# psipred/DMPfold2

Hardware: AMD Instinct MI355X
Metric: structures/s at L=300, N_seq=2000, 10 iters+100 min (higher is better)
Workload: dtype f32 with full-width operands on the bf16 matrix cores (option precision = 2): convolution operands split exactly into 3 bf16 pieces (24 significand bits), the 6 piece products above 2^-24 accumulated in f32 by v_mfma_f32_32x32x16_bf16; vertical GRU the same way (3 bf16 pieces per operand, 6 products

## Files before the change

### dmpfold2_amd/csrc/conv_bf16.h

```cpp
#pragma once
#include "common.h"
#include <vector>

namespace dmp {

typedef float cq_f32x16 __attribute__((ext_vector_type(16)));
typedef __bf16 cq_bf16x8 __attribute__((ext_vector_type(8)));

#ifndef CQ_PITCH_N
#define CQ_PITCH_N 20
#endif
constexpr int CQ_PITCH = CQ_PITCH_N;
constexpr int CQ_HCOLS = 20;
template <int NQ> struct CqShape {
  static constexpr int ROWS = 2 * NQ;
  static constexpr int HALO = ROWS + 4;
  static constexpr int RP = ROWS + 3;
  static constexpr int PIECE = 2 * HALO * CQ_PITCH;
  static constexpr int IN_SLOTS = 3 * PIECE;
  static constexpr int IN_PAD = (IN_SLOTS + 63) / 64 * 64;
  static constexpr int IN_BYTES = IN_PAD * 16;
};
constexpr int CQ_WSLOT = 3 * 2 * 32;
constexpr int CQ_WCOL = 5 * CQ_WSLOT;
constexpr int CQ_WBUF = 3 * CQ_WSLOT;
template <int NQ> constexpr int convq_lds_bytes() { return CqShape<NQ>::IN_BYTES + 4 * CQ_WBUF * 16; }
constexpr int CONVQ_LDS_BYTES = convq_lds_bytes<8>();

__host__ __device__ inline uint16_t cq_bf16_rne(float f) {
  uint32_t u = __builtin_bit_cast(uint32_t, f);
  u += 0x7FFFu + ((u >> 16) & 1u);
  return (uint16_t)(u >> 16);
}
__host__ __device__ inline float cq_bf16_f32(uint16_t h) {
  return __builtin_bit_cast(float, (uint32_t)h << 16);
}
__host__ __device__ inline void split3_bf16(float x, uint16_t p[3]) {
  p[0] = cq_bf16_rne(x);
  const float r1 = x - cq_bf16_f32(p[0]);
  p[1] = cq_bf16_rne(r1);
  const float r2 = r1 - cq_bf16_f32(p[1]);
  p[2] = cq_bf16_rne(r2);
}

inline std::vector<uint16_t> pack_conv_weights_bf16(const float* w) {
  const int tap_row[5] = {0, 2, 4, 1, 3};
  std::vector<uint16_t> q((size_t)4 * 8 * 25 * 4 * 3 * 2 * 32 * 8);
  for (int split = 0; split < 4; ++split)
    for (int g = 0; g < 8; ++g)
      for (int dx = 0; dx < 5; ++dx)
        for (int wave = 0; wave < 4; ++wave)
          for (int sl = 0; sl < 5; ++sl)
            for (int cg = 0; cg < 2; ++cg)
              for (int m = 0; m < 32; ++m)
                for (int e = 0; e < 8; ++e) {
                  const int oc = split * 128 + wave * 32 + m, ic = g * 16 + cg * 8 + e;
                  uint16_t p3[3];
                  split3_bf16(w[((size_t)oc * 128 + ic) * 25 + tap_row[sl] * 5 + dx], p3);
                  for (int p = 0; p < 3; ++p)
                    q[(((((((((size_t)split * 8 + g) * 5 + dx) * 4 + wave) * 5 + sl) * 3 + p) * 2 + cg) * 32 + m) * 8) + e] = p3[p];
                }
  return q;
}

#if defined(__HIPCC__) && defined(CONV_BF16_KERNELS)
__device__ __forceinline__ void cq_dma16(const void* gsrc, unsigned lds_byte_addr) {
  unsigned keep;
  asm volatile("s_mov_b32 %0, m0\n\ts_mov_b32 m0, %2\n\ts_nop 0\n\tglobal_load_lds_dwordx4 %1, off\n\ts_mov_b32 m0, %0"
               : "=&s"(keep) : "v"(gsrc), "s"(lds_byte_addr) : "memory");
}
template <int N> __device__ __forceinline__ void cq_wait_vm() {
  asm volatile("s_waitcnt vmcnt(%0)" :: "n"(N) : "memory");
}

__device__ __forceinline__ cq_f32x16 cq_mfma(uint4 a, uint4 b, cq_f32x16 c) {
  return __builtin_amdgcn_mfma_f32_32x32x16_bf16(__builtin_bit_cast(cq_bf16x8, a),
                                                 __builtin_bit_cast(cq_bf16x8, b), c, 0, 0, 0);
}

__device__ __forceinline__ void cq_lane_pixel(int li, int& row, int& x) {
  const bool a = li < 4 || (li >= 12 && li < 16) || (li >= 20 && li < 28);
  row = a ? 0 : 1;
  if (a) x = li < 4 ? li : (li < 16 ? li - 8 : li - 12);
  else x = li < 12 ? li - 4 : (li < 20 ? li - 8 : li - 16);
}

template <int NQ, int NT, int PAR>
__device__ __forceinline__ void cq_column_pass(const uint4 (&a)[NT][3], const uint4* il, cq_f32x16 (&acc)[NQ]) {
  constexpr int PIECE = CqShape<NQ>::PIECE, RP = CqShape<NQ>::RP;
  uint4 bn0 = il[PAR * CQ_PITCH], bn1 = il[PAR * CQ_PITCH + PIECE], bn2 = il[PAR * CQ_PITCH + 2 * PIECE];
#pragma unroll
  for (int r = PAR; r < RP; r += 2) {
    const uint4 b0 = bn0, b1 = bn1, b2 = bn2;
    if (r + 2 < RP) {
      bn0 = il[(r + 2) * CQ_PITCH];
      bn1 = il[(r + 2) * CQ_PITCH + PIECE];
      bn2 = il[(r + 2) * CQ_PITCH + 2 * PIECE];
    }
#define CQ_TAPS(AP, BV)                                                           \
    _Pragma("unroll") for (int t = 0; t < NT; ++t) {                              \
      const int q = (r - PAR - 2 * t) / 2;                                        \
      if (r - PAR - 2 * t >= 0 && q < NQ) acc[q] = cq_mfma(a[t][AP], BV, acc[q]); \
    }
    CQ_TAPS(0, b2)
    CQ_TAPS(1, b1)
    CQ_TAPS(2, b0)
    CQ_TAPS(0, b1)
    CQ_TAPS(1, b0)
    CQ_TAPS(0, b0)
#undef CQ_TAPS
  }
}

inline int conv_bf16_grid(int tiles, int bands = 1) {
  const int nt = tiles * tiles * bands;
  return 8 * ((nt + 1) / 2);
}

template <int NQ>
__global__ __launch_bounds__(256, 2) void conv5x5_bf16x6_kernel(const uint16_t* __restrict__ xs,
                                                                const uint16_t* __restrict__ wq,
                                                                const float* __restrict__ bias, int L, int P,
                                                                int tiles, int nwork, float* __restrict__ u,
                                                                double* __restrict__ part) {
  using SH = CqShape<NQ>;
  constexpr int BANDS = 8 / NQ;
  extern __shared__ __attribute__((aligned(16))) unsigned char cq_smem[];
  const int id = blockIdx.x;
  const int xcd = id & 7, slot = id >> 3;
  const int ntiles = tiles * tiles * BANDS;
  const int tper = (ntiles + 1) >> 1;
  const int tile = (xcd >> 2) * tper + slot;
  const int split = xcd & 3;
  if (slot >= tper || tile >= ntiles) return;
  const int trow = tile / tiles, tcol = tile % tiles;
  const int ty0 = trow * SH::ROWS, tx0 = tcol * CONV_TILE;
  const int tid = threadIdx.x, lane = tid & 63;
  const int wave = __builtin_amdgcn_readfirstlane(tid >> 6);
  const int kk = lane >> 5, li = lane & 31;
  const int64_t PP = (int64_t)P * P;
  const int64_t half0 = ((int64_t)(trow / BANDS) * tiles + tcol) * 2 + (trow % BANDS);
  if (BANDS == 2 && ty0 >= L) {
    if (li == 0)
      for (int g4 = 0; g4 < 4; ++g4) {
        const int gch = split * 32 + wave * 8 + 2 * g4 + kk;
        part[(half0 * CW + gch) * 2 + 0] = 0.0;
        part[(half0 * CW + gch) * 2 + 1] = 0.0;
      }
    return;
  }

  const uint4* in_l = reinterpret_cast<const uint4*>(cq_smem);
  const uint4* w_l = reinterpret_cast<const uint4*>(cq_smem + SH::IN_BYTES) + wave * CQ_WBUF;
  const unsigned lds_base = (unsigned)(size_t)(__attribute__((address_space(3))) unsigned char*)cq_smem;
  const unsigned w_lds_addr = lds_base + SH::IN_BYTES + wave * (CQ_WBUF * 16);

  const uint4* xs4 = reinterpret_cast<const uint4*>(xs);
  constexpr int NE = (SH::IN_PAD + 255) / 256;
  int in_src[NE];
#pragma unroll
  for (int e = 0; e < NE; ++e) {
    const int s = e * 256 + tid;
    const int sc = s < SH::IN_SLOTS ? s : 0;
    const int p = sc / SH::PIECE, r = sc % SH::PIECE;
    const int cg = r / (SH::HALO * CQ_PITCH), r2 = r % (SH::HALO * CQ_PITCH);
    const int yy = r2 / CQ_PITCH;
    int xx = r2 % CQ_PITCH;
    xx = xx < CQ_HCOLS ? xx : 0;
    in_src[e] = (int)(((int64_t)(p * 16 + cg) * P + ty0 + yy) * P + tx0 + xx);
  }
  const uint4* wq4 = reinterpret_cast<const uint4*>(wq) + (int64_t)split * 8 * 5 * 4 * CQ_WCOL +
                     (int64_t)wave * CQ_WCOL + lane;
  int prow, px;
  cq_lane_pixel(li, prow, px);
  const int b_base = (kk * SH::HALO + prow) * CQ_PITCH + px;
  const int a_off = kk * 32 + li;

  cq_f32x16 acc[NQ];
#pragma unroll
  for (int q = 0; q < NQ; ++q)
#pragma unroll
    for (int r = 0; r < 16; ++r) acc[q][r] = 0.f;

  auto wdma = [&](int h) {
    const int odd = h & 1;
    const uint4* src = wq4 + (int64_t)(h >> 1) * 4 * CQ_WCOL + odd * 3 * CQ_WSLOT;
    if (odd) {
#pragma unroll
      for (int i = 0; i < 6; ++i) cq_dma16(src + 64 * i, w_lds_addr + 1024 * i);
    } else {
#pragma unroll
      for (int i = 0; i < 9; ++i) cq_dma16(src + 64 * i, w_lds_addr + 1024 * i);
    }
  };
  wdma(0);

  for (int g = 0; g < 8; ++g) {
    __syncthreads();
    {
      const uint4* src = xs4 + (int64_t)g * 2 * PP;
      const unsigned dst = lds_base + (wave * 64) * 16;
#pragma unroll
      for (int e = 0; e < SH::IN_PAD / 256; ++e) cq_dma16(src + in_src[e], dst + e * 4096);
      if (wave * 64 < SH::IN_PAD % 256) cq_dma16(src + in_src[NE - 1], dst + (SH::IN_PAD / 256) * 4096);
    }
    cq_wait_vm<0>();
    __syncthreads();
#pragma unroll 1
    for (int dx = 0; dx < 5; ++dx) {
      const uint4* il = in_l + b_base + dx;
      const int h0 = 2 * (g * 5 + dx);
      {
        cq_wait_vm<0>();
        uint4 a[3][3];
#pragma unroll
        for (int t = 0; t < 3; ++t)
#pragma unroll
          for (int p = 0; p < 3; ++p) a[t][p] = w_l[t * CQ_WSLOT + p * 64 + a_off];
        asm volatile("s_waitcnt lgkmcnt(0)" ::: "memory");
        wdma(h0 + 1);
        cq_column_pass<NQ, 3, 0>(a, il, acc);
      }
      {
        cq_wait_vm<0>();
        uint4 a[2][3];
#pragma unroll
        for (int t = 0; t < 2; ++t)
#pragma unroll
          for (int p = 0; p < 3; ++p) a[t][p] = w_l[t * CQ_WSLOT + p * 64 + a_off];
        asm volatile("s_waitcnt lgkmcnt(0)" ::: "memory");
        if (h0 + 2 < 80) wdma(h0 + 2);
        cq_column_pass<NQ, 2, 1>(a, il, acc);
      }
    }
  }

  const float* bsp = bias + split * 128 + wave * 32;
  const int64_t LL = (int64_t)L * L;
#pragma unroll
  for (int g4 = 0; g4 < 4; ++g4) {
    const int cl = 8 * g4 + 4 * kk;
    const int gch = split * 32 + wave * 8 + 2 * g4 + kk;
    const float b0 = bsp[cl], b1 = bsp[cl + 1], b2 = bsp[cl + 2], b3 = bsp[cl + 3];
#pragma unroll
    for (int hq = 0; hq < NQ / 4; ++hq) {
      float s1 = 0.f, s2 = 0.f;
#pragma unroll
      for (int q = 4 * hq; q < 4 * hq + 4; ++q) {
        float v = acc[q][4 * g4] + b0;
        v = fmaxf(v, acc[q][4 * g4 + 1] + b1);
        v = fmaxf(v, acc[q][4 * g4 + 2] + b2);
        v = fmaxf(v, acc[q][4 * g4 + 3] + b3);
        const int y = ty0 + 2 * q + prow, x = tx0 + px;
        if (y < L && x < L) {
          u[(int64_t)gch * LL + (int64_t)y * L + x] = v;
          s1 += v;
          s2 += v * v;
        }
      }
#pragma unroll
      for (int off = 16; off > 0; off >>= 1) {
        s1 += __shfl_xor(s1, off, 32);
        s2 += __shfl_xor(s2, off, 32);
      }
      if (li == 0) {
        part[((half0 + hq) * CW + gch) * 2 + 0] = (double)s1;
        part[((half0 + hq) * CW + gch) * 2 + 1] = (double)s2;
      }
    }
  }
}
#endif

}
```

### dmpfold2_amd/csrc/trunk.hip

```cpp
#include "common.h"
#include <type_traits>
#define CONV_BF16_KERNELS
#include "conv_bf16.h"
#define CONV_F16_KERNELS
#include "conv_f16.h"

#pragma clang fp contract(off)

namespace dmp {

typedef float f32x16 __attribute__((ext_vector_type(16)));

__device__ __forceinline__ float sigmoid_f(float x) { return 1.0f / (1.0f + expf(-x)); }

template <int MODE>
__device__ __forceinline__ void store_pieces(const float (&o)[8], uint16_t* __restrict__ xs, int64_t slot,
                                             int64_t piece_stride, int* __restrict__ fault, float xscale) {
  constexpr int NP = (MODE == 0) ? 2 : 3;
  uint16_t pc[NP][8];
  bool bad = false;
#pragma unroll
  for (int e = 0; e < 8; ++e) {
    if constexpr (MODE == 0) {
      uint16_t p2[2];
      const float v = o[e] * xscale;
      split2_f16(v, p2);
      pc[0][e] = p2[0]; pc[1][e] = p2[1];
      bad = bad || !(fabsf(v) < 60000.f);
    } else {
      uint16_t p3[3];
      split3_bf16(o[e], p3);
      pc[0][e] = p3[0]; pc[1][e] = p3[1]; pc[2][e] = p3[2];
    }
  }
  if (bad) atomicOr(fault, 2);
#pragma unroll
  for (int p = 0; p < NP; ++p) {
    uint4 v;
    v.x = pc[p][0] | ((uint32_t)pc[p][1] << 16);
    v.y = pc[p][2] | ((uint32_t)pc[p][3] << 16);
    v.z = pc[p][4] | ((uint32_t)pc[p][5] << 16);
    v.w = pc[p][6] | ((uint32_t)pc[p][7] << 16);
    reinterpret_cast<uint4*>(xs)[p * piece_stride + slot] = v;
  }
}

__global__ __launch_bounds__(256) void act_pad_kernel(const float* __restrict__ dense, int L, int P,
                                                      float* __restrict__ xpad) {
  const int c = blockIdx.z, y = blockIdx.y;
  const int x = blockIdx.x * 256 + threadIdx.x;
  if (x >= P) return;
  const int yy = y - 2, xx = x - 2;
  float v = 0.f;
  if (yy >= 0 && yy < L && xx >= 0 && xx < L) v = dense[((int64_t)c * L + yy) * L + xx];
  xpad[((int64_t)c * P + y) * P + x] = v;
}

__global__ __launch_bounds__(256) void act_unpad_kernel(const float* __restrict__ xpad, int L, int P,
                                                        float* __restrict__ dense) {
  const int c = blockIdx.z, y = blockIdx.y;
  const int x = blockIdx.x * 256 + threadIdx.x;
  if (x >= L) return;
  dense[((int64_t)c * L + y) * L + x] = xpad[((int64_t)c * P + y + 2) * P + x + 2];
}

int act_pad(const float* d_dense, int L, float* d_xpad, hipStream_t s) {
  const int P = act_pitch(L);
  hipLaunchKernelGGL(act_pad_kernel, dim3(cdiv(P, 256), P, CW), dim3(256), 0, s, d_dense, L, P,
                     d_xpad);
  DMP_LAUNCH_CHECK();
  return DMP_OK;
}
int act_unpad(const float* d_xpad, int L, float* d_dense, hipStream_t s) {
  const int P = act_pitch(L);
  hipLaunchKernelGGL(act_unpad_kernel, dim3(cdiv(L, 256), L, CW), dim3(256), 0, s, d_xpad, L, P,
                     d_dense);
  DMP_LAUNCH_CHECK();
  return DMP_OK;
}
int act_clear(float* d_xpad, int L, hipStream_t s) {
  const int P = act_pitch(L);
  DMP_HIP(hipMemsetAsync(d_xpad, 0, sizeof(float) * CW * (size_t)P * P, s));
  return DMP_OK;
}

constexpr int SP_JT = 256;
__global__ __launch_bounds__(256) void stem_planes_kernel(const float* __restrict__ inv, int L,
                                                          float* __restrict__ planes) {
  __shared__ float row[SP_JT * NS];
  const int j0 = blockIdx.x * SP_JT, i = blockIdx.y, a = blockIdx.z;
  const int nj = min(SP_JT, L - j0);
  const int64_t D = (int64_t)L * NS, LL = (int64_t)L * L;
  const float* src = inv + ((int64_t)i * NS + a) * D + (int64_t)j0 * NS;
  for (int t = threadIdx.x; t < nj * NS; t += 256) row[t] = src[t];
  __syncthreads();
  const int j = threadIdx.x;
  if (j < nj) {
#pragma unroll
    for (int b = 0; b < NS; ++b) planes[(int64_t)(a * NS + b) * LL + (int64_t)i * L + j0 + j] = row[j * NS + b];
  }
}

constexpr int SS_CH = 8;
__global__ __launch_bounds__(256, 2) void stem_static_kernel(const float* __restrict__ wT,
                                                             const float* __restrict__ bias,
                                                             const float* __restrict__ m,
                                                             const float* __restrict__ planes, int L,
                                                             float* __restrict__ z0) {
  const int lane = threadIdx.x & 63, wave = threadIdx.x >> 6;
  const int kk = lane >> 5, li = lane & 31;
  const int64_t LL = (int64_t)L * L;
  const int64_t p0 = (int64_t)blockIdx.x * 64;
  const int64_t pq[2] = {p0 + li, p0 + 32 + li};
  const bool ok[2] = {pq[0] < LL, pq[1] < LL};
  const int64_t pc[2] = {ok[0] ? pq[0] : LL - 1, ok[1] ? pq[1] : LL - 1};
  const int iq[2] = {(int)(pc[0] / L), (int)(pc[1] / L)};
  const int jq[2] = {(int)(pc[0] - (int64_t)iq[0] * L), (int)(pc[1] - (int64_t)iq[1] * L)};

  f32x16 acc[3][2];
#pragma unroll
  for (int a = 0; a < 3; ++a)
#pragma unroll
    for (int q = 0; q < 2; ++q)
#pragma unroll
      for (int r = 0; r < 16; ++r) acc[a][q][r] = 0.f;

  const unsigned woff = 4u * (unsigned)(kk * STEM_OUT + wave * 96 + li);
  const unsigned moff_i[2] = {4u * (unsigned)(kk * L + iq[0]), 4u * (unsigned)(kk * L + iq[1])};
  const unsigned moff_j[2] = {4u * (unsigned)(kk * L + jq[0]), 4u * (unsigned)(kk * L + jq[1])};
  const unsigned poff[2] = {4u * (unsigned)(kk * LL + pc[0]), 4u * (unsigned)(kk * LL + pc[1])};
  constexpr int NCH1 = WIDTH / 2 / SS_CH;
  const int npairs = planes ? (STEM_IN - 1) / 2 : WIDTH / 2;
  const int nchunks = (npairs + SS_CH - 1) / SS_CH;
  const __amdgpu_buffer_rsrc_t wrs = __builtin_amdgcn_make_buffer_rsrc(const_cast<float*>(wT), 0, (STEM_IN - 1) * STEM_OUT * 4, 0x00020000);
  const __amdgpu_buffer_rsrc_t mrs = __builtin_amdgcn_make_buffer_rsrc(const_cast<float*>(m), 0, WIDTH * L * 4, 0x00020000);
  auto ldb = [](__amdgpu_buffer_rsrc_t r, unsigned voff, unsigned soff) {
    return __builtin_bit_cast(float, __builtin_amdgcn_raw_buffer_load_b32(r, voff, soff, 0));
  };
  float av[2][SS_CH][3], r0[2][SS_CH][2], r1[2][SS_CH][2];
  using B0 = std::integral_constant<int, 0>;
  using B1 = std::integral_constant<int, 1>;
  auto load1 = [&](auto BUF, int c) {
    constexpr int buf = decltype(BUF)::value;
#pragma unroll
    for (int u = 0; u < SS_CH; ++u) {
      const unsigned k2 = 2u * (unsigned)(c * SS_CH + u);
#pragma unroll
      for (int x = 0; x < 3; ++x) av[buf][u][x] = ldb(wrs, woff + 128u * x, k2 * (STEM_OUT * 4u));
#pragma unroll
      for (int q = 0; q < 2; ++q) {
        r0[buf][u][q] = ldb(mrs, moff_i[q], k2 * (4u * (unsigned)L));
        r1[buf][u][q] = ldb(mrs, moff_j[q], k2 * (4u * (unsigned)L));
      }
    }
  };
  auto load2 = [&](auto BUF, int c) {
    constexpr int buf = decltype(BUF)::value;
    const int k0 = 2 * c * SS_CH;
    const int live_k = min(2 * SS_CH, 2 * npairs - k0);
    const __amdgpu_buffer_rsrc_t prs = __builtin_amdgcn_make_buffer_rsrc(
        const_cast<float*>(planes) + (int64_t)(k0 - WIDTH) * LL, 0, (int)((int64_t)live_k * LL * 4), 0x00020000);
    const __amdgpu_buffer_rsrc_t wr2 = __builtin_amdgcn_make_buffer_rsrc(
        const_cast<float*>(wT) + (int64_t)k0 * STEM_OUT, 0, live_k * STEM_OUT * 4, 0x00020000);
#pragma unroll
    for (int u = 0; u < SS_CH; ++u) {
#pragma unroll
      for (int x = 0; x < 3; ++x) av[buf][u][x] = ldb(wr2, woff + 128u * x, 2u * u * (STEM_OUT * 4u));
#pragma unroll
      for (int q = 0; q < 2; ++q) r0[buf][u][q] = ldb(prs, poff[q], 2u * u * (4u * (unsigned)LL));
    }
  };
  auto compute = [&](auto BUF, auto PHASE) {
    constexpr int buf = decltype(BUF)::value;
#pragma unroll
    for (int u = 0; u < SS_CH; ++u) {
      float b0 = r0[buf][u][0], b1 = r0[buf][u][1];
      if (decltype(PHASE)::value == 1) { b0 *= r1[buf][u][0]; b1 *= r1[buf][u][1]; }
      b0 = ok[0] ? b0 : 0.f;
      b1 = ok[1] ? b1 : 0.f;
#pragma unroll
      for (int a = 0; a < 3; ++a) {
        acc[a][0] = __builtin_amdgcn_mfma_f32_32x32x2f32(av[buf][u][a], b0, acc[a][0], 0, 0, 0);
        acc[a][1] = __builtin_amdgcn_mfma_f32_32x32x2f32(av[buf][u][a], b1, acc[a][1], 0, 0, 0);
      }
    }
  };
  using P1 = std::integral_constant<int, 1>;
  using P2 = std::integral_constant<int, 2>;
  load1(B0{}, 0);
#pragma unroll 1
  for (int c = 0; c < NCH1; c += 2) {
    load1(B1{}, c + 1);
    __builtin_amdgcn_sched_barrier(0);
    compute(B0{}, P1{});
    __builtin_amdgcn_sched_barrier(0);
    if (c + 2 < NCH1) load1(B0{}, c + 2);
    else if (c + 2 < nchunks) load2(B0{}, c + 2);
    __builtin_amdgcn_sched_barrier(0);
    compute(B1{}, P1{});
    __builtin_amdgcn_sched_barrier(0);
  }
#pragma unroll 1
  for (int c = NCH1; c < nchunks; c += 2) {
    if (c + 1 < nchunks) load2(B1{}, c + 1);
    __builtin_amdgcn_sched_barrier(0);
    compute(B0{}, P2{});
    __builtin_amdgcn_sched_barrier(0);
    if (c + 1 < nchunks) {
      if (c + 2 < nchunks) load2(B0{}, c + 2);
      __builtin_amdgcn_sched_barrier(0);
      compute(B1{}, P2{});
      __builtin_amdgcn_sched_barrier(0);
    }
  }
#pragma unroll
  for (int a = 0; a < 3; ++a)
#pragma unroll
    for (int q = 0; q < 2; ++q) {
      if (!ok[q]) continue;
#pragma unroll
      for (int r = 0; r < 16; ++r) {
        const int o = wave * 96 + a * 32 + (r & 3) + 8 * (r >> 2) + 4 * kk;
        z0[(int64_t)o * LL + pq[q]] = acc[a][q][r] + bias[o];
      }
    }
}

int stem_static(dmp_ctx* c, const float* d_mat1d, const float* d_inv, const float* d_contacts,
                int L, float* d_z0, hipStream_t s) {
  const Weights& W = c->W;
  const int64_t LL = (int64_t)L * L;
  const float* planes = nullptr;
  if (d_inv != nullptr) {
    hipLaunchKernelGGL(stem_planes_kernel, dim3(cdiv(L, SP_JT), L, NS), dim3(256), 0, s, d_inv, L, c->planes);
    DMP_LAUNCH_CHECK();
    DMP_HIP(hipMemcpyAsync(c->planes + (int64_t)NS * NS * LL, d_contacts, sizeof(float) * LL, hipMemcpyDeviceToDevice, s));
    planes = c->planes;
  }
  hipLaunchKernelGGL(stem_static_kernel, dim3((unsigned)cdiv64(LL, 64)), dim3(256), 0, s, W.stemT, W.stem_b,
                     d_mat1d, planes, L, d_z0);
  DMP_LAUNCH_CHECK();
  return DMP_OK;
}

__global__ __launch_bounds__(256) void stem_maxout_kernel(const float* __restrict__ z0,
                                                          const float* __restrict__ wd,
                                                          const float* __restrict__ dmap, int64_t LL,
                                                          float* __restrict__ u, double* __restrict__ part) {
  __shared__ double red[2][4];
  const int64_t p = (int64_t)blockIdx.x * 256 + threadIdx.x;
  const int g = blockIdx.y;
  double s1 = 0.0, s2 = 0.0;
  if (p < LL) {
    const float d = dmap[p];
    const float v0 = z0[(int64_t)(3 * g) * LL + p] + wd[3 * g] * d;
    const float v1 = z0[(int64_t)(3 * g + 1) * LL + p] + wd[3 * g + 1] * d;
    const float v2 = z0[(int64_t)(3 * g + 2) * LL + p] + wd[3 * g + 2] * d;
    const float v = fmaxf(fmaxf(v0, v1), v2);
    u[(int64_t)g * LL + p] = v;
    s1 = (double)v;
    s2 = s1 * s1;
  }
  s1 = wave_sum_f64(s1);
  s2 = wave_sum_f64(s2);
  if ((threadIdx.x & 63) == 0) { red[0][threadIdx.x >> 6] = s1; red[1][threadIdx.x >> 6] = s2; }
  __syncthreads();
  if (threadIdx.x < 2) {
    const double t = ((red[threadIdx.x][0] + red[threadIdx.x][1]) + red[threadIdx.x][2]) + red[threadIdx.x][3];
    part[((int64_t)blockIdx.x * CW + g) * 2 + threadIdx.x] = t;
  }
}

__global__ __launch_bounds__(64) void stats_reduce_kernel(const double* __restrict__ part, int nparts,
                                                          double* __restrict__ stats, double count,
                                                          const float* __restrict__ gamma,
                                                          const float* __restrict__ beta,
                                                          float* __restrict__ ab) {
  const int c = blockIdx.x;
  double s1 = 0.0, s2 = 0.0;
  for (int t = threadIdx.x; t < nparts; t += 64) {
    s1 += part[((int64_t)t * CW + c) * 2 + 0];
    s2 += part[((int64_t)t * CW + c) * 2 + 1];
  }
  for (int off = 32; off > 0; off >>= 1) {
    s1 += __shfl_xor(s1, off, 64);
    s2 += __shfl_xor(s2, off, 64);
  }
  if (threadIdx.x == 0) {
    stats[c * 2 + 0] = s1;
    stats[c * 2 + 1] = s2;
    if (ab) {
      const double mean = s1 / count;
      double var = s2 / count - mean * mean;
      var = var < 0.0 ? 0.0 : var;
      const float invstd = (float)(1.0 / sqrt(var + 1e-5));
      const float alpha = invstd * gamma[c];
      ab[c * 2 + 0] = alpha;
      ab[c * 2 + 1] = beta[c] - (float)mean * alpha;
    }
  }
}

__global__ void norm_coeff_kernel(const double* __restrict__ stats, double count,
                                  const float* __restrict__ gamma, const float* __restrict__ beta,
                                  float* __restrict__ ab) {
  const int c = threadIdx.x;
  const double mean = stats[c * 2] / count;
  double var = stats[c * 2 + 1] / count - mean * mean;
  var = var < 0.0 ? 0.0 : var;
  const float invstd = (float)(1.0 / sqrt(var + 1e-5));
  const float alpha = invstd * gamma[c];
  ab[c * 2 + 0] = alpha;
  ab[c * 2 + 1] = beta[c] - (float)mean * alpha;
}

template <int SPLIT>
__global__ __launch_bounds__(256) void stem_norm_kernel(const float* __restrict__ u,
                                                        const float* __restrict__ ab, int L, int P,
                                                        float* __restrict__ xpad, uint16_t* __restrict__ xs,
                                                        int* __restrict__ fault, float xscale) {
  const int y = blockIdx.y, cgp = blockIdx.z;
  const int x = blockIdx.x * 256 + threadIdx.x;
  if (x >= P) return;
  const int yy = y - 2, xx = x - 2;
  const bool inside = yy >= 0 && yy < L && xx >= 0 && xx < L;
  if (SPLIT < 0 && !inside) return;
  const int64_t PP = (int64_t)P * P, LL = (int64_t)L * L;
  float o[8];
#pragma unroll
  for (int e = 0; e < 8; ++e) {
    const int c = cgp * 8 + e;
    o[e] = 0.f;
    if (inside) {
      o[e] = u[(int64_t)c * LL + (int64_t)yy * L + xx] * ab[c * 2] + ab[c * 2 + 1];
      xpad[(int64_t)c * PP + (int64_t)y * P + x] = o[e];
    }
  }
  if constexpr (SPLIT == 0) store_pieces<0>(o, xs, (int64_t)cgp * PP + (int64_t)y * P + x, 16 * PP, fault, xscale);
  if constexpr (SPLIT == 2) store_pieces<2>(o, xs, (int64_t)cgp * PP + (int64_t)y * P + x, 16 * PP, fault, 1.0f);
}

int stem_update_padded(dmp_ctx* c, const float* d_z0, const float* d_dmap, int L, float* d_xpad,
                       hipStream_t s, bool split) {
  const Weights& W = c->W;
  const int64_t LL = (int64_t)L * L;
  const int P = act_pitch(L);
  const unsigned nblk = (unsigned)cdiv64(LL, 256);
  hipLaunchKernelGGL(stem_maxout_kernel, dim3(nblk, CW), dim3(256), 0, s, d_z0,
                     W.stem_wd, d_dmap, LL, c->u, c->part);
  DMP_LAUNCH_CHECK();
  hipLaunchKernelGGL(stats_reduce_kernel, dim3(CW), dim3(64), 0, s, c->part, (int)nblk, c->stats, (double)LL,
                     W.stem_gamma, W.stem_beta, c->ab);
  DMP_LAUNCH_CHECK();
  const dim3 grid(cdiv(P, 256), P, 16);
  const int mode = (split && c->conv_mode != 1) ? c->conv_mode : -1;
  if (mode == 0)
    hipLaunchKernelGGL(stem_norm_kernel<0>, grid, dim3(256), 0, s, c->u, c->ab, L, P, d_xpad, c->xsplit, c->seq_abort,
                       c->act_scaling ? W.blk[0].x_scale : 1.0f);
  else if (mode == 2)
    hipLaunchKernelGGL(stem_norm_kernel<2>, grid, dim3(256), 0, s, c->u, c->ab, L, P, d_xpad, c->xsplit, c->seq_abort, 1.0f);
  else
    hipLaunchKernelGGL(stem_norm_kernel<-1>, grid, dim3(256), 0, s, c->u, c->ab, L, P, d_xpad, (uint16_t*)nullptr,
                       c->seq_abort, 1.0f);
  DMP_LAUNCH_CHECK();
  return DMP_OK;
}

constexpr int HALO = CONV_TILE + 4;
constexpr int IN_PITCH = 24;
constexpr int NTAP = 25;
constexpr int MCH = 128;
constexpr int NCHUNK = CW / CONV_CC;
constexpr int W_STAGE = NTAP * CONV_CC * MCH;
constexpr int IN_STAGE = CONV_CC * HALO * IN_PITCH;

template <bool IDX>
__global__ __launch_bounds__(256, 2) void conv5x5_maxout_kernel(const float* __restrict__ xpad,
                                                                const float* __restrict__ wpack,
                                                                const float* __restrict__ bias, int L,
                                                                int P, int tiles, int nwork,
                                                                float* __restrict__ u,
                                                                double* __restrict__ part,
                                                                uint8_t* __restrict__ idx) {
  __shared__ __attribute__((aligned(16))) float smem[2 * W_STAGE + 2 * IN_STAGE];
  float (*w_lds)[W_STAGE] = reinterpret_cast<float (*)[W_STAGE]>(smem);
  float (*in_lds)[IN_STAGE] = reinterpret_cast<float (*)[IN_STAGE]>(smem + 2 * W_STAGE);
  constexpr int IP = IN_PITCH;
  const int id = blockIdx.x;
  const int per = gridDim.x >> 3;
  const int work = (id & 7) * per + (id >> 3);
  if (work >= nwork) return;
  const int tile = work >> 2, split = work & 3;
  const int ty0 = (tile / tiles) * CONV_TILE, tx0 = (tile % tiles) * CONV_TILE;

  const int tid = threadIdx.x, lane = tid & 63, wave = tid >> 6;
  const int kk = lane >> 5, li = lane & 31;
  const int64_t PP = (int64_t)P * P;

  const float4* wsrc = reinterpret_cast<const float4*>(wpack + (int64_t)split * NCHUNK * W_STAGE);
  int in_off[4], in_dst[4];
  bool in_ok[4];
#pragma unroll
  for (int e = 0; e < 4; ++e) {
    const int idx = tid + e * 256;
    in_ok[e] = idx < CONV_CC * HALO * HALO;
    const int idc = in_ok[e] ? idx : 0;
    const int cc = idc / (HALO * HALO), rem = idc % (HALO * HALO);
    const int yy = rem / HALO, xx = rem % HALO;
    in_off[e] = (int)(cc * PP + (int64_t)(ty0 + yy) * P + tx0 + xx);
    in_dst[e] = cc * HALO * IP + yy * IP + xx;
  }
  float ireg[4];
  auto prefetch = [&](int chunk) {
    const float4* ws = wsrc + (int64_t)chunk * (W_STAGE / 4);
    const float* xs = xpad + (int64_t)chunk * CONV_CC * PP;
    typedef __attribute__((address_space(1))) const void* gptr_t;
    typedef __attribute__((address_space(3))) void* lptr_t;
    float* dst = w_lds[(chunk & 1)] + (size_t)wave * 256;
#pragma unroll
    for (int e = 0; e < 6; ++e)
      __builtin_amdgcn_global_load_lds((gptr_t)(ws + tid + e * 256), (lptr_t)(dst + e * 1024), 16, 0, 0);
    if (wave == 0)
      __builtin_amdgcn_global_load_lds((gptr_t)(ws + tid + 6 * 256), (lptr_t)(dst + 6 * 1024), 16, 0, 0);
#pragma unroll
    for (int e = 0; e < 4; ++e) ireg[e] = xs[in_off[e]];
  };
  auto commit = [&](int buf) {
#pragma unroll
    for (int e = 0; e < 4; ++e)
      if (in_ok[e]) in_lds[buf][in_dst[e]] = ireg[e];
  };

  int b_off[2];
#pragma unroll
  for (int q = 0; q < 2; ++q) {
    const int nb = 2 * wave + q;
    const int y = (nb >> 1) * 4 + (li >> 3), x = (nb & 1) * 8 + (li & 7);
    b_off[q] = kk * HALO * IP + y * IP + x;
  }
  const int a_off = kk * MCH + li;

  f32x16 acc[4][2];
#pragma unroll
  for (int mb = 0; mb < 4; ++mb)
#pragma unroll
    for (int q = 0; q < 2; ++q)
#pragma unroll
      for (int r = 0; r < 16; ++r) acc[mb][q][r] = 0.f;

  prefetch(0);
  commit(0);
  __syncthreads();
  for (int chunk = 0; chunk < NCHUNK; ++chunk) {
    const int buf = chunk & 1;
    if (chunk + 1 < NCHUNK) prefetch(chunk + 1);
    const float* wl = w_lds[buf] + a_off;
    const float* il = in_lds[buf];
#pragma unroll
    for (int tap = 0; tap < NTAP; ++tap) {
      const int dy = tap / 5, dx = tap % 5;
      float a[4], b[2];
#pragma unroll
      for (int mb = 0; mb < 4; ++mb) a[mb] = wl[tap * CONV_CC * MCH + mb * 32];
#pragma unroll
      for (int q = 0; q < 2; ++q) b[q] = il[b_off[q] + dy * IP + dx];
#pragma unroll
      for (int mb = 0; mb < 4; ++mb)
#pragma unroll
        for (int q = 0; q < 2; ++q)
          acc[mb][q] = __builtin_amdgcn_mfma_f32_32x32x2f32(a[mb], b[q], acc[mb][q], 0, 0, 0);
    }
    if (chunk + 1 < NCHUNK) commit(buf ^ 1);
    __syncthreads();
  }

  float* sred = w_lds[0];
  const float* bsp = bias + split * MCH;
  const int64_t LL = (int64_t)L * L;
#pragma unroll
  for (int mb = 0; mb < 4; ++mb)
#pragma unroll
    for (int g4 = 0; g4 < 4; ++g4) {
      const int cl = mb * 32 + 8 * g4 + 4 * kk;
      const int gch = split * 32 + (cl >> 2);
      float s1 = 0.f, s2 = 0.f;
#pragma unroll
      for (int q = 0; q < 2; ++q) {
        float v = acc[mb][q][4 * g4] + bsp[cl];
        int win = 0;
        if constexpr (IDX) {
#pragma unroll
          for (int e = 1; e < 4; ++e) {
            const float t = acc[mb][q][4 * g4 + e] + bsp[cl + e];
            if (t > v) { v = t; win = e; }
          }
        } else {
          v = fmaxf(v, acc[mb][q][4 * g4 + 1] + bsp[cl + 1]);
          v = fmaxf(v, acc[mb][q][4 * g4 + 2] + bsp[cl + 2]);
          v = fmaxf(v, acc[mb][q][4 * g4 + 3] + bsp[cl + 3]);
        }
        const int nb = 2 * wave + q;
        const int y = ty0 + (nb >> 1) * 4 + (li >> 3), x = tx0 + (nb & 1) * 8 + (li & 7);
        if (y < L && x < L) {
          if constexpr (IDX) idx[(int64_t)gch * LL + (int64_t)y * L + x] = (uint8_t)win;
          u[(int64_t)gch * LL + (int64_t)y * L + x] = v;
          s1 += v;
          s2 += v * v;
        }
      }
#pragma unroll
      for (int off = 16; off > 0; off >>= 1) {
        s1 += __shfl_xor(s1, off, 32);
        s2 += __shfl_xor(s2, off, 32);
      }
      if (li == 0) {
        const int chl = (cl >> 2);
        sred[(wave * 32 + chl) * 2 + 0] = s1;
        sred[(wave * 32 + chl) * 2 + 1] = s2;
      }
    }
  __syncthreads();
  if (tid < 64) {
    const int chl = tid >> 1, which = tid & 1;
    double t = 0.0;
#pragma unroll
    for (int wv = 0; wv < 4; ++wv) t += (double)sred[(wv * 32 + chl) * 2 + which];
    part[((int64_t)tile * CW + split * 32 + chl) * 2 + which] = t;
  }
}

int conv5x5_reduce_stats(dmp_ctx* c, int L, double* d_stats, hipStream_t s, int block) {
  const int nparts = c->part_count;
  if (block > 0) {
    const BlockW& B = c->W.blk[block - 1];
    hipLaunchKernelGGL(stats_reduce_kernel, dim3(CW), dim3(64), 0, s, c->part, nparts, d_stats,
                       (double)L * (double)L, B.gamma, B.beta, c->ab);
    c->ab_current = true;
  } else {
    hipLaunchKernelGGL(stats_reduce_kernel, dim3(CW), dim3(64), 0, s, c->part, nparts, d_stats, 1.0,
                       (const float*)nullptr, (const float*)nullptr, (float*)nullptr);
  }
  DMP_LAUNCH_CHECK();
  return DMP_OK;
}

template <int MODE>
__global__ __launch_bounds__(256) void act_split_kernel(const float* __restrict__ xpad, int P,
                                                        uint16_t* __restrict__ xs, int* __restrict__ fault,
                                                        float xscale) {
  const int y = blockIdx.y, cgp = blockIdx.z;
  const int x = blockIdx.x * 256 + threadIdx.x;
  if (x >= P) return;
  const int64_t PP = (int64_t)P * P;
  float o[8];
#pragma unroll
  for (int e = 0; e < 8; ++e) o[e] = xpad[(int64_t)(cgp * 8 + e) * PP + (int64_t)y * P + x];
  store_pieces<MODE>(o, xs, (int64_t)cgp * PP + (int64_t)y * P + x, 16 * PP, fault, xscale);
}

int act_split(dmp_ctx* c, const float* d_xpad, int L, int block, hipStream_t s) {
  const int P = act_pitch(L);
  dim3 grid(cdiv(P, 256), P, 16);
  if (c->conv_mode == 2)
    hipLaunchKernelGGL(act_split_kernel<2>, grid, dim3(256), 0, s, d_xpad, P, c->xsplit, c->seq_abort, 1.0f);
  else
    hipLaunchKernelGGL(act_split_kernel<0>, grid, dim3(256), 0, s, d_xpad, P, c->xsplit, c->seq_abort,
                       c->act_scaling ? c->W.blk[block - 1].x_scale : 1.0f);
  DMP_LAUNCH_CHECK();
  return DMP_OK;
}

int trunk_kernel_attrs(dmp_ctx* c) {
  static bool done[64] = {};
  if (c->device >= 0 && c->device < 64 && done[c->device]) return DMP_OK;
  DMP_HIP(hipFuncSetAttribute((const void*)conv5x5_bf16x6_kernel<8>, hipFuncAttributeMaxDynamicSharedMemorySize,
                              convq_lds_bytes<8>()));
  DMP_HIP(hipFuncSetAttribute((const void*)conv5x5_bf16x6_kernel<4>, hipFuncAttributeMaxDynamicSharedMemorySize,
                              convq_lds_bytes<4>()));
  DMP_HIP(hipFuncSetAttribute((const void*)conv5x5_f16x3_kernel<8>, hipFuncAttributeMaxDynamicSharedMemorySize,
                              convh_lds_bytes<8>()));
  DMP_HIP(hipFuncSetAttribute((const void*)conv5x5_f16x3_kernel<4>, hipFuncAttributeMaxDynamicSharedMemorySize,
                              convh_lds_bytes<4>()));
  if (c->device >= 0 && c->device < 64) done[c->device] = true;
  return DMP_OK;
}

int conv5x5_maxout_padded(dmp_ctx* c, int block, const float* d_xpad, int L, float* d_u,
                          double* d_stats, hipStream_t s, bool reduce) {
  const BlockW& B = c->W.blk[block - 1];
  const int tiles = act_tiles(L), P = act_pitch(L);
  const int nwork = tiles * tiles * CONV_SPLIT;
  const int grid = round_up(nwork, 8);
  if (c->conv_mode != 1) {
    if (!c->xsplit_current) {
      int rc = act_split(c, d_xpad, L, block, s);
      if (rc) return rc;
    }
    const int bands = c->conv_tile_bands > 0 ? c->conv_tile_bands : conv_split_rows(tiles);
    const float scale = c->act_scaling ? B.wh_inv_scale / B.x_scale : B.wh_inv_scale;
    if (c->conv_mode == 2) {
      if (bands == 2)
        hipLaunchKernelGGL(conv5x5_bf16x6_kernel<4>, dim3(conv_bf16_grid(tiles, 2)), dim3(256), convq_lds_bytes<4>(), s,
                           c->xsplit, B.wq, B.bias, L, P, tiles, nwork, d_u, c->part);
      else
        hipLaunchKernelGGL(conv5x5_bf16x6_kernel<8>, dim3(conv_bf16_grid(tiles, 1)), dim3(256), convq_lds_bytes<8>(), s,
                           c->xsplit, B.wq, B.bias, L, P, tiles, nwork, d_u, c->part);
    } else {
      if (bands == 2)
        hipLaunchKernelGGL(conv5x5_f16x3_kernel<4>, dim3(conv_f16_grid(tiles, 2)), dim3(256), convh_lds_bytes<4>(), s,
                           c->xsplit, B.wh, B.bias, scale, L, P, tiles, nwork, d_u, c->part);
      else
        hipLaunchKernelGGL(conv5x5_f16x3_kernel<8>, dim3(conv_f16_grid(tiles, 1)), dim3(256), convh_lds_bytes<8>(), s,
                           c->xsplit, B.wh, B.bias, scale, L, P, tiles, nwork, d_u, c->part);
    }
    DMP_LAUNCH_CHECK();
    c->part_count = 2 * tiles * tiles;
    return reduce ? conv5x5_reduce_stats(c, L, d_stats, s) : DMP_OK;
  }
  hipLaunchKernelGGL(conv5x5_maxout_kernel<false>, dim3(grid), dim3(256), 0, s, d_xpad, B.wpack, B.bias, L,
                     P, tiles, nwork, d_u, c->part, (uint8_t*)nullptr);
  DMP_LAUNCH_CHECK();
  c->part_count = tiles * tiles;
  return reduce ? conv5x5_reduce_stats(c, L, d_stats, s) : DMP_OK;
}

int conv5x5_maxout_winners(dmp_ctx* c, int block, const float* d_xpad, int L, float* d_u, uint8_t* d_idx, hipStream_t s) {
  const BlockW& B = c->W.blk[block - 1];
  const int tiles = act_tiles(L), P = act_pitch(L);
  const int nwork = tiles * tiles * CONV_SPLIT;
  hipLaunchKernelGGL(conv5x5_maxout_kernel<true>, dim3(round_up(nwork, 8)), dim3(256), 0, s, d_xpad, B.wpack, B.bias, L,
                     P, tiles, nwork, d_u, c->part, d_idx);
  DMP_LAUNCH_CHECK();
  c->part_count = tiles * tiles;
  return DMP_OK;
}

#ifndef NORM_PRIO
#define NORM_PRIO 0
#endif
template <int SPLIT, int HEAD>
__global__ __launch_bounds__(256) void norm_scse_residual_kernel(
    const float* __restrict__ u, const float* __restrict__ ab, const float* __restrict__ cse,
    const float* __restrict__ sse_w, float sse_b, const float* __restrict__ xin, int L, int P,
    float* __restrict__ xout, uint16_t* __restrict__ xs, int* __restrict__ fault, float xscale,
    const float* __restrict__ hw, float hb0, float hb1, float* __restrict__ head0, float* __restrict__ head1) {
  __shared__ float sh_a[CW], sh_b[CW], sh_g[CW], sh_w[CW], sh_h[HEAD ? 2 * CW : 1];
#if NORM_PRIO
  __builtin_amdgcn_s_setprio(NORM_PRIO);
#endif
  if (threadIdx.x < CW) {
    sh_a[threadIdx.x] = ab[threadIdx.x * 2];
    sh_b[threadIdx.x] = ab[threadIdx.x * 2 + 1];
    sh_g[threadIdx.x] = cse[threadIdx.x];
    sh_w[threadIdx.x] = sse_w[threadIdx.x];
  }
  if constexpr (HEAD) sh_h[threadIdx.x] = hw[threadIdx.x];
  __syncthreads();
  const int lane = threadIdx.x & 63, wave = threadIdx.x >> 6;
  const int q = lane >> 4;
  const int y = blockIdx.y;
  const int x = blockIdx.x * 64 + wave * 16 + (lane & 15);
  const bool live = x < L;
  const int xc = live ? x : L - 1;
  const int64_t LL = (int64_t)L * L, PP = (int64_t)P * P;
  const int64_t p = (int64_t)y * L + xc, pp = (int64_t)(y + 2) * P + xc + 2;
  constexpr int QC = CW / 4;
  float yv[QC];
  float dot = 0.f;
#pragma unroll
  for (int i = 0; i < QC; ++i) {
    const int c = q * QC + i;
    yv[i] = u[c * LL + p] * sh_a[c] + sh_b[c];
    dot = fmaf(sh_w[c], yv[i], dot);
  }
  dot += __shfl_xor(dot, 16, 64);
  dot += __shfl_xor(dot, 32, 64);
  const float sg = sigmoid_f(dot + sse_b);
  float h0 = 0.f, h1 = 0.f;
#pragma unroll
  for (int g8 = 0; g8 < QC / 8; ++g8) {
    const int cgp = q * (QC / 8) + g8;
    float o[8];
#pragma unroll
    for (int e = 0; e < 8; ++e) {
      const int c = cgp * 8 + e;
      const float t = yv[g8 * 8 + e] * sh_g[c] + yv[g8 * 8 + e] * sg;
      o[e] = t + xin[c * PP + pp];
      if (live) xout[c * PP + pp] = o[e];
      if constexpr (HEAD) {
        h0 = fmaf(sh_h[c], o[e], h0);
        h1 = fmaf(sh_h[CW + c], o[e], h1);
      }
    }
    if (live) {
      if constexpr (SPLIT == 0) store_pieces<0>(o, xs, (int64_t)cgp * PP + pp, 16 * PP, fault, xscale);
      if constexpr (SPLIT == 2) store_pieces<2>(o, xs, (int64_t)cgp * PP + pp, 16 * PP, fault, 1.0f);
    }
  }
  if constexpr (HEAD) {
    h0 += __shfl_xor(h0, 16, 64);
    h0 += __shfl_xor(h0, 32, 64);
    h1 += __shfl_xor(h1, 16, 64);
    h1 += __shfl_xor(h1, 32, 64);
    if (live && q == 0) {
      head0[(int64_t)y * L + x] = h0 + hb0;
      head1[(int64_t)y * L + x] = h1 + hb1;
    }
  }
}

int norm_scse_residual_padded(dmp_ctx* c, int block, const float* d_u, const double* d_stats,
                              const float* d_xpad_in, int L, float* d_xpad_out, hipStream_t s, bool head) {
  const BlockW& B = c->W.blk[block - 1];
  const Weights& W = c->W;
  const int P = act_pitch(L);
  if (!c->ab_current) {
    hipLaunchKernelGGL(norm_coeff_kernel, dim3(1), dim3(CW), 0, s, d_stats, (double)L * (double)L,
                       B.gamma, B.beta, c->ab);
    DMP_LAUNCH_CHECK();
  }
  c->ab_current = false;
  const int split = (c->conv_mode != 1 && c->xsplit_current && block < NBLOCK) ? c->conv_mode : -1;
  const float xscale = (c->act_scaling && block < NBLOCK) ? c->W.blk[block].x_scale : 1.0f;
  dim3 grid(cdiv(L, 64), L);
#define NORM_LAUNCH(S, H)                                                                              \
  hipLaunchKernelGGL((norm_scse_residual_kernel<S, H>), grid, dim3(256), 0, s, d_u, c->ab, B.cse, B.sse_w, \
                     B.sse_b, d_xpad_in, L, P, d_xpad_out, c->xsplit, c->seq_abort, xscale, W.head_w,   \
                     W.head_b[0], W.head_b[1], c->head0, c->head1)
  if (head) NORM_LAUNCH(-1, 1);
  else if (split == 0) NORM_LAUNCH(0, 0);
  else if (split == 2) NORM_LAUNCH(2, 0);
  else NORM_LAUNCH(-1, 0);
#undef NORM_LAUNCH
  DMP_LAUNCH_CHECK();
  c->head_current = head;
  return DMP_OK;
}

__global__ __launch_bounds__(256) void head_planes_kernel(const float* __restrict__ xpad,
                                                          const float* __restrict__ hw, float b0, float b1,
                                                          int L, int P, float* __restrict__ head0,
                                                          float* __restrict__ head1) {
  __shared__ float sw[2 * CW];
  sw[threadIdx.x] = hw[threadIdx.x];
  __syncthreads();
  const int i = blockIdx.y;
  const int j = blockIdx.x * 256 + threadIdx.x;
  if (j >= L) return;
  const int64_t PP = (int64_t)P * P;
  const float* px = xpad + (int64_t)(i + 2) * P + j + 2;
  float p0[4], p1[4];
#pragma unroll
  for (int q = 0; q < 4; ++q) {
    p0[q] = 0.f; p1[q] = 0.f;
#pragma unroll 8
    for (int k = 0; k < CW / 4; ++k) {
      const int c = q * (CW / 4) + k;
      const float v = px[c * PP];
      p0[q] = fmaf(sw[c], v, p0[q]);
      p1[q] = fmaf(sw[CW + c], v, p1[q]);
    }
  }
  head0[(int64_t)i * L + j] = ((p0[0] + p0[1]) + (p0[2] + p0[3])) + b0;
  head1[(int64_t)i * L + j] = ((p1[0] + p1[1]) + (p1[2] + p1[3])) + b1;
}

__global__ __launch_bounds__(256) void head_conf_kernel(const float* __restrict__ head1, int L,
                                                        float* __restrict__ conf) {
  __shared__ double red[256];
  const int i = blockIdx.x;
  double rsum = 0.0;
  for (int j = threadIdx.x; j < L; j += 256) rsum += (double)head1[(int64_t)i * L + j];
  const double total = block_tree_sum_f64<256>(rsum, red);
  if (threadIdx.x == 0) conf[i] = (float)(total / (double)L);
}

__global__ __launch_bounds__(256) void gram_kernel(const float* __restrict__ h0, int L,
                                                   float* __restrict__ M) {
  const int i = blockIdx.y;
  const int j = blockIdx.x * 256 + threadIdx.x;
  if (j >= L) return;
  auto dm = [&](int a, int b) {
    return distmap_entry(h0[(int64_t)a * L + b], h0[(int64_t)b * L + a]);
  };
  const float d0j = dm(0, j), di0 = dm(i, 0), dij = dm(i, j);
  const float t = d0j * d0j + di0 * di0;
  M[(int64_t)i * L + j] = 0.5f * (t - dij * dij);
}

int head_gram_padded(dmp_ctx* c, const float* d_xpad, int L, float* d_conf, float* d_M,
                     hipStream_t s) {
  const Weights& W = c->W;
  const int P = act_pitch(L);
  if (!c->head_current) {
    hipLaunchKernelGGL(head_planes_kernel, dim3(cdiv(L, 256), L), dim3(256), 0, s, d_xpad, W.head_w, W.head_b[0],
                       W.head_b[1], L, P, c->head0, c->head1);
    DMP_LAUNCH_CHECK();
  }
  c->head_current = false;
  hipLaunchKernelGGL(head_conf_kernel, dim3(L), dim3(256), 0, s, c->head1, L, d_conf);
  DMP_LAUNCH_CHECK();
  hipLaunchKernelGGL(gram_kernel, dim3(cdiv(L, 256), L), dim3(256), 0, s, c->head0, L, d_M);
  DMP_LAUNCH_CHECK();
  return DMP_OK;
}

}
```

Measured before the change: 4.173.

## Double-buffer conv input tiles in LDS and load weights directly to registers

The conv kernel now keeps two LDS input-tile buffers and issues the DMA for the next channel group partway through the first column pass, so the global-to-LDS transfer overlaps MFMA work. Before, each group synchronised, loaded, then waited. Weights no longer go through per-wave LDS staging with DMA. They are read from global memory straight into registers, prefetched one half-column ahead of use. This adds register pressure and LDS use (two tiles), which could lower occupancy under launch_bounds(256,2). It also adds an optional clock-stamp probe behind a macro.

```diff
diff --git a/dmpfold2_amd/csrc/conv_bf16.h b/dmpfold2_amd/csrc/conv_bf16.h
--- a/dmpfold2_amd/csrc/conv_bf16.h
+++ b/dmpfold2_amd/csrc/conv_bf16.h
@@ -23,8 +23,7 @@
 };
 constexpr int CQ_WSLOT = 3 * 2 * 32;
 constexpr int CQ_WCOL = 5 * CQ_WSLOT;
-constexpr int CQ_WBUF = 3 * CQ_WSLOT;
-template <int NQ> constexpr int convq_lds_bytes() { return CqShape<NQ>::IN_BYTES + 4 * CQ_WBUF * 16; }
+template <int NQ> constexpr int convq_lds_bytes() { return 2 * CqShape<NQ>::IN_BYTES; }
 constexpr int CONVQ_LDS_BYTES = convq_lds_bytes<8>();
 
 __host__ __device__ inline uint16_t cq_bf16_rne(float f) {
@@ -85,8 +84,8 @@
   else x = li < 12 ? li - 4 : (li < 20 ? li - 8 : li - 16);
 }
 
-template <int NQ, int NT, int PAR>
-__device__ __forceinline__ void cq_column_pass(const uint4 (&a)[NT][3], const uint4* il, cq_f32x16 (&acc)[NQ]) {
+template <int NQ, int NT, int PAR, class MID>
+__device__ __forceinline__ void cq_column_pass(const uint4 (&a)[NT][3], const uint4* il, cq_f32x16 (&acc)[NQ], MID&& mid) {
   constexpr int PIECE = CqShape<NQ>::PIECE, RP = CqShape<NQ>::RP;
   uint4 bn0 = il[PAR * CQ_PITCH], bn1 = il[PAR * CQ_PITCH + PIECE], bn2 = il[PAR * CQ_PITCH + 2 * PIECE];
 #pragma unroll
@@ -109,8 +108,22 @@
     CQ_TAPS(1, b0)
     CQ_TAPS(0, b0)
 #undef CQ_TAPS
-  }
-}
+    if (r == PAR + 2 * (NT - 1)) mid();
+  }
+}
+
+template <int NT>
+__device__ __forceinline__ void cq_load_weights(const uint4* __restrict__ src, uint4 (&a)[NT][3]) {
+#pragma unroll
+  for (int t = 0; t < NT; ++t)
+#pragma unroll
+    for (int p = 0; p < 3; ++p) a[t][p] = src[t * CQ_WSLOT + p * 64];
+}
+
+#ifdef CQ_CLOCK_STAMPS
+constexpr int CQ_STAMP_BLOCKS = 2048;
+__device__ unsigned long long cq_clock_stamps[CQ_STAMP_BLOCKS][2];
+#endif
 
 inline int conv_bf16_grid(int tiles, int bands = 1) {
   const int nt = tiles * tiles * bands;
@@ -151,9 +164,7 @@
   }
 
   const uint4* in_l = reinterpret_cast<const uint4*>(cq_smem);
-  const uint4* w_l = reinterpret_cast<const uint4*>(cq_smem + SH::IN_BYTES) + wave * CQ_WBUF;
   const unsigned lds_base = (unsigned)(size_t)(__attribute__((address_space(3))) unsigned char*)cq_smem;
-  const unsigned w_lds_addr = lds_base + SH::IN_BYTES + wave * (CQ_WBUF * 16);
 
   const uint4* xs4 = reinterpret_cast<const uint4*>(xs);
   constexpr int NE = (SH::IN_PAD + 255) / 256;
@@ -169,12 +180,18 @@
     xx = xx < CQ_HCOLS ? xx : 0;
     in_src[e] = (int)(((int64_t)(p * 16 + cg) * P + ty0 + yy) * P + tx0 + xx);
   }
-  const uint4* wq4 = reinterpret_cast<const uint4*>(wq) + (int64_t)split * 8 * 5 * 4 * CQ_WCOL +
-                     (int64_t)wave * CQ_WCOL + lane;
+  auto tile_dma = [&](int g) {
+    const uint4* src = xs4 + (int64_t)g * 2 * PP;
+    const unsigned dst = lds_base + (g & 1) * SH::IN_BYTES + (wave * 64) * 16;
+#pragma unroll
+    for (int e = 0; e < SH::IN_PAD / 256; ++e) cq_dma16(src + in_src[e], dst + e * 4096);
+    if (wave * 64 < SH::IN_PAD % 256) cq_dma16(src + in_src[NE - 1], dst + (SH::IN_PAD / 256) * 4096);
+  };
+  const uint4* wcol = reinterpret_cast<const uint4*>(wq) + (int64_t)split * 8 * 5 * 4 * CQ_WCOL +
+                      (int64_t)wave * CQ_WCOL + lane;
   int prow, px;
   cq_lane_pixel(li, prow, px);
   const int b_base = (kk * SH::HALO + prow) * CQ_PITCH + px;
-  const int a_off = kk * 32 + li;
 
   cq_f32x16 acc[NQ];
 #pragma unroll
@@ -182,58 +199,49 @@
 #pragma unroll
     for (int r = 0; r < 16; ++r) acc[q][r] = 0.f;
 
-  auto wdma = [&](int h) {
-    const int odd = h & 1;
-    const uint4* src = wq4 + (int64_t)(h >> 1) * 4 * CQ_WCOL + odd * 3 * CQ_WSLOT;
-    if (odd) {
-#pragma unroll
-      for (int i = 0; i < 6; ++i) cq_dma16(src + 64 * i, w_lds_addr + 1024 * i);
-    } else {
-#pragma unroll
-      for (int i = 0; i < 9; ++i) cq_dma16(src + 64 * i, w_lds_addr + 1024 * i);
-    }
-  };
-  wdma(0);
+  uint4 ae[3][3], ao[2][3];
+  tile_dma(0);
+  cq_load_weights<3>(wcol, ae);
+  __builtin_amdgcn_sched_barrier(0);
+#ifdef CQ_CLOCK_STAMPS
+  const unsigned long long st_clk = __builtin_amdgcn_s_memtime(), st_real = __builtin_amdgcn_s_memrealtime();
+#endif
 
   for (int g = 0; g < 8; ++g) {
-    __syncthreads();
-    {
-      const uint4* src = xs4 + (int64_t)g * 2 * PP;
-      const unsigned dst = lds_base + (wave * 64) * 16;
-#pragma unroll
-      for (int e = 0; e < SH::IN_PAD / 256; ++e) cq_dma16(src + in_src[e], dst + e * 4096);
-      if (wave * 64 < SH::IN_PAD % 256) cq_dma16(src + in_src[NE - 1], dst + (SH::IN_PAD / 256) * 4096);
-    }
     cq_wait_vm<0>();
     __syncthreads();
+    const uint4* in_g = in_l + (g & 1) * SH::IN_PAD + b_base;
 #pragma unroll 1
     for (int dx = 0; dx < 5; ++dx) {
-      const uint4* il = in_l + b_base + dx;
-      const int h0 = 2 * (g * 5 + dx);
+      const uint4* il = in_g + dx;
       {
-        cq_wait_vm<0>();
-        uint4 a[3][3];
-#pragma unroll
-        for (int t = 0; t < 3; ++t)
-#pragma unroll
-          for (int p = 0; p < 3; ++p) a[t][p] = w_l[t * CQ_WSLOT + p * 64 + a_off];
-        asm volatile("s_waitcnt lgkmcnt(0)" ::: "memory");
-        wdma(h0 + 1);
-        cq_column_pass<NQ, 3, 0>(a, il, acc);
+        __builtin_amdgcn_sched_barrier(0);
+        cq_load_weights<2>(wcol + 3 * CQ_WSLOT, ao);
+        __builtin_amdgcn_sched_barrier(0);
+        cq_column_pass<NQ, 3, 0>(ae, il, acc, [&] {
+          if (dx == 0 && g < 7) {
+            __builtin_amdgcn_sched_barrier(0);
+            tile_dma(g + 1);
+            __builtin_amdgcn_sched_barrier(0);
+          }
+        });
       }
       {
-        cq_wait_vm<0>();
-        uint4 a[2][3];
-#pragma unroll
-        for (int t = 0; t < 2; ++t)
-#pragma unroll
-          for (int p = 0; p < 3; ++p) a[t][p] = w_l[t * CQ_WSLOT + p * 64 + a_off];
-        asm volatile("s_waitcnt lgkmcnt(0)" ::: "memory");
-        if (h0 + 2 < 80) wdma(h0 + 2);
-        cq_column_pass<NQ, 2, 1>(a, il, acc);
-      }
-    }
-  }
+        const uint4* wnext = wcol + (g * 5 + dx < 39 ? 4 * CQ_WCOL : 0);
+        __builtin_amdgcn_sched_barrier(0);
+        cq_load_weights<3>(wnext, ae);
+        __builtin_amdgcn_sched_barrier(0);
+        cq_column_pass<NQ, 2, 1>(ao, il, acc, [] {});
+        wcol = wnext;
+      }
+    }
+  }
+#ifdef CQ_CLOCK_STAMPS
+  if (tid == 0 && id < CQ_STAMP_BLOCKS) {
+    cq_clock_stamps[id][0] = __builtin_amdgcn_s_memtime() - st_clk;
+    cq_clock_stamps[id][1] = __builtin_amdgcn_s_memrealtime() - st_real;
+  }
+#endif
 
   const float* bsp = bias + split * 128 + wave * 32;
   const int64_t LL = (int64_t)L * L;
diff --git a/dmpfold2_amd/csrc/trunk.hip b/dmpfold2_amd/csrc/trunk.hip
--- a/dmpfold2_amd/csrc/trunk.hip
+++ b/dmpfold2_amd/csrc/trunk.hip
@@ -806,3 +806,11 @@
 }
 
 }
+
+#ifdef CQ_CLOCK_STAMPS
+extern "C" int dmp_debug_conv_clock(unsigned long long* host, int blocks) {
+  if (!host || blocks < 1 || blocks > dmp::CQ_STAMP_BLOCKS) return -1;
+  if (hipDeviceSynchronize() != hipSuccess) return -1;
+  return hipMemcpyFromSymbol(host, HIP_SYMBOL(dmp::cq_clock_stamps), sizeof(unsigned long long) * 2 * blocks) == hipSuccess ? 0 : -1;
+}
+#endif
```

After: 4.364, median of 6. 1.05x the previous value.
